# Nick-qsv/MLP-PPO-2PLY-P3

Hardware: AMD Instinct MI355X
Metric: self-play env steps/sec (whole node) + 2-ply evals/sec at batch=65536 (higher is better)
Workload: dtype int8 boards / fp32-equivalent policy MLP (split-f16 MFMA); 1 GPU; C3: B=65536 games/GPU PPO rollout step (policy 198->128->{500,1} + masked sample + env.step, rollout rows stored to an HBM ring); global_batch=65536, games_per_gpu=65536, max_legal_moves=500, parallelism=dp1 (independent game shards), streams_per_gpu=4, step_fork=False

## Files before the change

mlp-ppo-2ply-p3_amd/csrc/bg_engine.h:

```cpp
#pragma once
#include <hip/hip_runtime.h>
#include <stdint.h>
#include <stdlib.h>
#include <string>

#include "bg_core.h"
#include "../../include/bgx.h"

namespace bg {

template <int LOG> constexpr int cap_fast() { return (7 << LOG) / 8; }
constexpr int kLogSlotsSlow = 17;
constexpr int kCapSlow = (7 << kLogSlotsSlow) / 8;
constexpr int kSlowWaves = 32;
constexpr int kMtWords = 640;

constexpr int R_CUR = 52, R_ROLL0 = 53, R_ROLL1 = 54, R_OVER = 55, R_MATCH = 56, R_S0 = 57, R_S1 = 58,
              R_NEED = 59, R_NM0 = 60, R_NM1 = 61, R_FLAGS = 62;
constexpr int NEED_NONE = 0, NEED_ROLL = 1, NEED_RESET = 2;

__device__ __forceinline__ int lane_id() { return threadIdx.x & 63; }
__device__ __forceinline__ int rd(int bv, int i) { return __builtin_amdgcn_readlane(bv, i); }
__device__ __forceinline__ int wr(int bv, int i, int v) { return lane_id() == i ? v : bv; }
__device__ __forceinline__ uint32_t ufl(uint32_t v) { return __builtin_amdgcn_readfirstlane(v); }
// ... 78 lines not shown
            #pragma unroll
            for (int r = 0; r < 10; ++r) {
                const uint32_t h0 = __umulhi(0xD2511F53u, c0), l0 = 0xD2511F53u * c0;
                const uint32_t h1 = __umulhi(0xCD9E8D57u, c2), l1 = 0xCD9E8D57u * c2;
                c0 = h1 ^ c1 ^ a0; c1 = l1; c2 = h0 ^ c3 ^ a1; c3 = l0;
                a0 += 0x9E3779B9u; a1 += 0xBB67AE85u;
            }
            blk0 = c0; blk1 = c1; blk2 = c2; blk3 = c3; blkid = b;
        }
        const uint32_t w = (uint32_t)(ctr & 3u);
        ++ctr;
        return w == 0 ? blk0 : w == 1 ? blk1 : w == 2 ? blk2 : blk3;
    }

    template <bool PHILOX_ONLY = false>
    __device__ int die() {
        used = true;
        for (;;) {
            const uint32_t x = (PHILOX_ONLY || mode == BGX_DICE_PHILOX ? next_philox() : next_mt()) & 7u;
            if (x <= 5u) return (int)x + 1;
        }
    }

    template <bool PHILOX_ONLY = false>
    __device__ void finish(uint64_t* ctr_out) {
        if (!used) return;
        if (PHILOX_ONLY || mode == BGX_DICE_PHILOX) {
            if (lane_id() == 0) *ctr_out = ctr;
            return;
        }
        if (twisted) {
            for (int j = lane_id(); j < 624; j += 64) mt[j] = sh[j];
        }
        if (lane_id() == 0) mt[624] = (uint32_t)idx;
    }
};

struct Args {
    uint8_t* lanes;
    uint64_t* moves;
    int32_t* n_total;
    uint32_t* mt;
    uint64_t* ctr;
    uint8_t* shared_rolls;
    int32_t* ovf_count;
    int32_t* ovf_queue;
    int32_t* err;
    int B, max_moves, dice_mode, auto_reset, match_length;
    uint32_t key0, key1;
    uint64_t* stamps;
    int cap_mid;
    int cap_main;
    int32_t* perm;
    uint8_t* cls;
    uint8_t* pre;
    int xcd;
    const uint8_t* starts;
};
constexpr int kStartOk = 63;

__device__ __forceinline__ int lane_of_block(const Args& A, int bi) {
    if (!A.xcd) return bi;
    const int r = bi & 127;
    return (bi & ~127) | ((r & 7) << 4) | (r >> 3);
}

constexpr int kClasses = 5;

constexpr uint64_t kCtrMask = (1ull << 48) - 1ull;

constexpr int kPreOver = 0x80;
__device__ __forceinline__ int pre_class(int bv) {
    if (rd(bv, R_OVER)) return kPreOver;
    const int nxt = 1 - rd(bv, R_CUR);
    const int l = lane_id();
    const int off = nxt * 24;
    const bool mine = l >= off && l < off + 24 && bv > 0;
    return __popcll(__ballot(mine)) + (rd(bv, 48 + nxt) > 0 ? 2 : 0);
}

__device__ __forceinline__ int predict_class(int pre, uint64_t ctr, uint32_t key0, uint32_t key1, uint32_t lane_no,
                                             uint32_t& cache) {
    cache = 0u;
    if (pre & kPreOver) return kClasses - 1;
    Rng r;
    const uint64_t c0 = ctr & kCtrMask;
    r.init_philox(c0, key0, key1, lane_no);
    const int a = r.die(), b = r.die();
    const uint64_t draws = r.ctr - c0;
    if (draws < 32) cache = 0x8000u | (uint32_t)a | ((uint32_t)b << 3) | ((uint32_t)draws << 6);
    if (a != b) return kClasses - 1;
    const int pts = pre;
    if (pts >= 10 && a <= 4) return 0;
    if ((pts >= 8 && a <= 5) || pts >= 10) return 1;
    return pts >= 5 ? 2 : 3;
}

template <int LOG, typename SlotPtr, int MEMO_KIND = 0, bool NO_DOUBLES = false>
__device__ __forceinline__ int run_movegen(int bv, int pl, int r0, int r1, uint64_t* out, int cap, SlotPtr tab,
                                           int cap_unique, int* total, bool* ovf, uint4* memo) {
    const bool dbl = r0 == r1;
    Gen<LOG, SlotPtr, MoveSink, MEMO_KIND> g;
    g.tab = tab; g.sink.out = out; g.sink.cap = cap; g.pl = pl; g.cap_unique = cap_unique;
    g.memo2 = memo && dbl ? memo : nullptr;
    g.memo3 = memo && dbl ? (MEMO_KIND != 0 ? memo : memo + (1 << kLogMemo2)) : nullptr;
    uint32_t blocked;
    const Node s0 = node_from_bytes(bv, pl, blocked);
    g.blocked = blocked;
    if (NO_DOUBLES) g.run_nd(s0, r0, r1);
    else g.run(s0, r0, r1);
    *ovf = g.ovf;
    *total = g.count;
    return g.count < cap ? g.count : cap;
}

template <int DICE = -1>
__device__ __forceinline__ bool roll_lane(int& bv, int gi, const Args& A, uint32_t* mt_scratch, uint64_t* ctr_io,
                                          int& r0, int& r1) {
    const int need = rd(bv, R_NEED);
    if (need == NEED_NONE) return false;
// ... 75 lines not shown
}

__device__ __forceinline__ int defer_lane(int bv, int gi, const Args& A) {
    if (lane_id() == 0) { const int q = atomicAdd(A.ovf_count, 1); A.ovf_queue[q] = gi; A.n_total[gi] = 0; }
    bv = wr(bv, R_NM0, 0);
    bv = wr(bv, R_NM1, 0);
    bv = wr(bv, R_FLAGS, rd(bv, R_FLAGS) | 1);
    return wr(bv, R_NEED, NEED_NONE);
}

template <int LOG, int MEMO_KIND = 0, bool NO_DOUBLES = false, int DICE = -1>
__device__ __forceinline__ int advance_lane(int bv, int gi, const Args& A, uint4* lds_tab, uint4* lds_memo,
                                            uint64_t* ctr_io) {
    int r0, r1;
    if (!roll_lane<DICE>(bv, gi, A, (uint32_t*)lds_tab, ctr_io, r0, r1)) return bv;
    if (NO_DOUBLES && r0 == r1) return defer_lane(bv, gi, A);
    return movegen_lane<LOG, MEMO_KIND, NO_DOUBLES>(bv, gi, A, r0, r1, lds_tab, lds_memo);
}

__device__ __forceinline__ void write_obs(int bv, float* obs_row) {
    const int cur = rd(bv, R_CUR);
    #pragma unroll
    for (int t = 0; t < 4; ++t) {
        const int f = lane_id() + 64 * t;
        const float v = feature_at(bv, f < 198 ? f : 197, cur);
        if (f < 198) obs_row[f] = v;
    }
}

__device__ __forceinline__ int apply_move_bytes(int bv, uint32_t mlo, uint32_t mhi, int pl) {
    mlo = opaque(mlo); mhi = opaque(mhi);
    const int l = lane_id();
    const uint32_t q = (uint32_t)(l - pl * 24);
    const uint32_t o = (uint32_t)(l - (24 - pl * 24));
    constexpr uint32_t kNone = 32u;
    const uint32_t my_src = q < 24u ? q : (l == 48 + pl ? (uint32_t)kBar : kNone);
    const uint32_t my_dst = q < 24u ? q : (l == 50 + pl ? (uint32_t)kOff : kNone);
    uint32_t ok = 1u, hits = 0u;
    int delta = 0;
    #pragma unroll
    for (int i = 0; i < 4; ++i) {
        const uint32_t e = (i < 2 ? mlo : mhi) >> (16 * (i & 1));
        ok &= e >> 15;
        const uint32_t src = e & 31u, dst = (e >> 5) & 31u;
        const int d = (int)(dst == my_dst) - (int)(src == my_src);
        delta += ok ? d : 0;
        hits |= (ok & (e >> 10)) << dst;
    }
    if (o < 24u) delta -= (int)((hits >> o) & 1u);
    if (l == 49 - pl) delta += __popc(hits);
    return bv + delta;
}

__device__ __forceinline__ int apply_lane(int bv, int gi, int action, const Args& A, float* reward, uint8_t* done,
                                          int32_t* info) {
    const int mover = rd(bv, R_CUR);
    int winner = -1, score = 0, kind = 0, dn = 0;
    float rew = 0.0f;
    if (rd(bv, R_OVER)) {
        bv = wr(bv, R_NEED, NEED_RESET);
        dn = 1; kind = 3;
    } else {
        const int n = rd(bv, R_NM0) | (rd(bv, R_NM1) << 8);
        if (n == 0) {
            bv = wr(bv, R_CUR, 1 - mover);
            bv = wr(bv, R_NEED, NEED_ROLL);
            kind = 1;
        } else {
            const int a = action < 0 ? action + A.max_moves : action;
            if (a < 0 || a >= n) {
                rew = -1.0f; kind = 2;
            } else {
                const uint64_t mv = A.moves[(size_t)gi * A.max_moves + a];
                bv = apply_move_bytes(bv, (uint32_t)mv, (uint32_t)(mv >> 32), mover);
                if (rd(bv, 50 + mover) == 15) {
                    const int opp = 1 - mover;
                    const bool opp_off0 = rd(bv, 50 + opp) == 0;
                    const int l = lane_id();
                    const int hl = mover == 0 ? 18 : 0;
                    const bool in_home = l >= opp * 24 + hl && l < opp * 24 + hl + 6 && bv > 0;
                    const bool bg = opp_off0 && (__ballot(in_home) != 0ull || rd(bv, 48 + opp) > 0);
                    score = bg ? 3 : (opp_off0 ? 2 : 1);
                    rew = bg ? 2.0f : (opp_off0 ? 1.5f : 1.0f);
                    winner = mover; dn = 1;
                    const int ns = rd(bv, R_S0 + mover) + score;
                    bv = wr(bv, R_S0 + mover, ns > 255 ? 255 : ns);
                    bv = wr(bv, R_OVER, 1);
                    if (ns >= A.match_length) bv = wr(bv, R_MATCH, 1);
                    if (A.auto_reset) bv = wr(bv, R_NEED, NEED_RESET);
                } else {
                    bv = wr(bv, R_CUR, 1 - mover);
                    bv = wr(bv, R_NEED, NEED_ROLL);
                }
            }
        }
    }
    if (lane_id() == 0) {
        reward[gi] = rew;
        done[gi] = (uint8_t)dn;
        if (info) info[gi] = mover | ((winner + 1) << 8) | (score << 16) | (kind << 24);
    }
    return bv;
}

__device__ __forceinline__ int load_rec(const Args& A, int gi) { return (int)A.lanes[(size_t)gi * 64 + lane_id()]; }
__device__ __forceinline__ void store_rec(const Args& A, int gi, int bv) { A.lanes[(size_t)gi * 64 + lane_id()] = (uint8_t)bv; }


}

struct DeviceBuf {
    void* p = nullptr;
    size_t cap = 0;
    hipError_t reserve(size_t bytes, int slack_num, hipStream_t stream, size_t keep_bytes) {
        if (cap >= bytes) return hipSuccess;
        hipError_t err = hipStreamSynchronize(stream);
        if (err != hipSuccess) return err;
        const size_t ncap = bytes + bytes * (size_t)slack_num / 100;
        void* np = nullptr;
        if ((err = hipMalloc(&np, ncap)) != hipSuccess) return err;
        if (p && keep_bytes) {
            err = hipMemcpyAsync(np, p, keep_bytes, hipMemcpyDeviceToDevice, stream);
            if (err == hipSuccess) err = hipStreamSynchronize(stream);
            if (err != hipSuccess) { (void)hipFree(np); return err; }
        }
        void* old = p;
        p = np;
        cap = ncap;
        return old ? hipFree(old) : hipSuccess;
    }
};

struct bgx_engine {
    bool step_debug{false};
    int device{0};
    bg::Args a{};
    uint4* slow_tables{nullptr};
    int slow_waves{bg::kSlowWaves};
    int32_t* perm{nullptr};
    bool perm_valid{false};
    int32_t* order_cnt{nullptr};
    hipStream_t step_side{nullptr};
    hipEvent_t step_ev[4]{};
    bool order_pending{false};
    bool step_fork{true};
    int32_t* ovf_base{nullptr};
    int ovf_parity{0};
    bool ovf_next_zeroed{false};
    uint64_t seed{0};
    uint8_t* starts{nullptr};
    DeviceBuf search_ws;
    DeviceBuf search_pool;
    hipStream_t search_side{nullptr};
    hipEvent_t search_ev[5]{};
    float search_ms[2]{};
    DeviceBuf oneply_ws;
    hipEvent_t use_ev{nullptr};
    hipStream_t use_stream{nullptr};
    bool use_valid{false};
};

inline hipError_t join_order(bgx_engine* e, hipStream_t s) {
    if (!e->order_pending) return hipSuccess;
    const hipError_t err = hipStreamWaitEvent(s, e->step_ev[3], 0);
    if (err == hipSuccess) e->order_pending = false;
    return err;
}

struct EngineCall {
    bgx_engine* e;
    hipStream_t s;
    bool entered = false, captured = false;
    hipError_t err;
    EngineCall(bgx_engine* e_, hipStream_t s_, bool join = false) : e(e_), s(s_), err(hipSetDevice(e_->device)) {
        if (err != hipSuccess) return;
        entered = true;
        hipStreamCaptureStatus cs = hipStreamCaptureStatusNone;
        if (hipStreamIsCapturing(s, &cs) == hipSuccess && cs != hipStreamCaptureStatusNone) captured = true;
        if (!captured && e->use_valid && e->use_stream != s) err = hipStreamWaitEvent(s, e->use_ev, 0);
        if (err == hipSuccess && join) err = join_order(e, s);
    }
    ~EngineCall() {
        if (!entered) return;
        if (captured) { e->use_valid = false; return; }
        if (!e->use_ev && hipEventCreateWithFlags(&e->use_ev, hipEventDisableTiming) != hipSuccess) {
            e->use_ev = nullptr;
            e->use_valid = false;
            return;
        }
        e->use_valid = hipEventRecord(e->use_ev, s) == hipSuccess;
        e->use_stream = s;
    }
};
// ... 1 lines not shown
```

mlp-ppo-2ply-p3_amd/csrc/bg_engine.hip:

```cpp
#include <hip/hip_runtime.h>
#include <stdio.h>
#include <stdint.h>
#include <string.h>
#include <stdlib.h>
#include <algorithm>
#include <cmath>
#include <mutex>
#include <string>
#include <vector>

#include "bg_engine.h"
#include "bg_rollout.h"
#include "bg_debug.h"
#include "bg_host.h"
#include <map>

using namespace bg;

namespace {

constexpr int kMaxRegions = BGX_MAX_COPY_REGIONS;
using namespace bg;

template <int PHASE, int LOG, int MEMO, bool NO_DOUBLES = false, int DICE = -1>
__device__ __forceinline__ void step_lane(const Args& A, int gi, uint4* tab, uint4* memo, const int32_t* actions,
                                          float* obs, float* reward, uint8_t* done, int32_t* info) {
    const uint64_t t0 = A.stamps ? __builtin_amdgcn_s_memrealtime() : 0;
    int bv = load_rec(A, gi);
    const int act = PHASE != 2 ? (int)ufl((uint32_t)actions[gi]) : 0;
    uint64_t ctr = (DICE >= 0 ? DICE : A.dice_mode) == BGX_DICE_PHILOX ? A.ctr[gi] : 0;
    if (PHASE != 2) bv = apply_lane(bv, gi, act, A, reward, done, info);
    if (PHASE != 1) {
        bv = advance_lane<LOG, MEMO == 2 ? 2 : 0, NO_DOUBLES, DICE>(bv, gi, A, tab, memo, &ctr);
        if (obs) write_obs(bv, obs + (size_t)gi * 198);
    }
    store_rec(A, gi, bv);
    if (PHASE == 0 && A.pre) {
        const int p = pre_class(bv);
        if (lane_id() == 0) A.pre[gi] = (uint8_t)p;
    }
    if (A.stamps && lane_id() == 0) {
        A.stamps[2 * gi] = t0;
        A.stamps[2 * gi + 1] = __builtin_amdgcn_s_memrealtime();
    }
}

template <int PHASE, int LOG, int MEMO = 1, bool NO_DOUBLES = false, int WPE = 1, int DICE = -1>
__global__ __launch_bounds__(64) __attribute__((amdgpu_waves_per_eu(WPE))) void k_step(Args A, const int32_t* actions, float* obs, float* reward, uint8_t* done,
                                             int32_t* info, int base) {
    __shared__ uint4 tab[1 << LOG];
    __shared__ uint4 memo_[MEMO == 1 ? kMemoSlots : 1];
    uint4* memo = MEMO == 1 ? memo_ : MEMO == 2 ? tab : nullptr;
    const int bi = (int)blockIdx.x + base;
    const int gi = A.perm ? (int)ufl((uint32_t)A.perm[bi]) : lane_of_block(A, bi);
    step_lane<PHASE, LOG, MEMO, NO_DOUBLES, DICE>(A, gi, tab, memo, actions, obs, reward, done, info);
}

template <int LOG>
__global__ __launch_bounds__(64) void k_reset(Args A, const uint8_t* lane_mask, float* obs, int mark_only) {
    __shared__ uint4 tab[1 << LOG];
    __shared__ uint4 memo[kMemoSlots];
    const int gi = blockIdx.x;
    int bv = load_rec(A, gi);
    uint64_t ctr = A.dice_mode == BGX_DICE_PHILOX ? A.ctr[gi] : 0;
    const bool sel = lane_mask == nullptr || ufl(lane_mask[gi]) != 0u;
    if (sel) bv = wr(bv, R_NEED, NEED_RESET);
    if (!mark_only) {
        bv = advance_lane<LOG>(bv, gi, A, tab, memo, &ctr);
        if (obs) write_obs(bv, obs + (size_t)gi * 198);
        if (A.pre) {
            const int p = pre_class(bv);
            if (lane_id() == 0) A.pre[gi] = (uint8_t)p;
        }
    }
    store_rec(A, gi, bv);
}

constexpr int kXcd = 8, kRun = 16;
__device__ __forceinline__ int order_class(const uint8_t* cls, int i, int B) {
    return i < B ? min((int)cls[i], kClasses - 1) : kClasses;
}

constexpr int kCountThreads = 256;
__global__ __launch_bounds__(kCountThreads) void k_order_count(const uint8_t* pre, uint8_t* cls, uint64_t* ctr, uint32_t key0,
                                                      uint32_t key1, int32_t* cnt, int B, int32_t* zero_next,
                                                      int xcd) {
    __shared__ int sc[kXcd][kClasses];
    const int t = threadIdx.x, i = blockIdx.x * kCountThreads + t, w = t >> 6;
    if (blockIdx.x == 0 && t < 4) zero_next[t] = 0;
    if (t < kXcd * kClasses) sc[t / kClasses][t % kClasses] = 0;
    __syncthreads();
    int c = kClasses;
    if (i < B) {
        const int p = (int)pre[i];
        const uint64_t cv = (p & kPreOver) ? 0ull : ctr[i];
        uint32_t cache;
        c = predict_class(p, cv, key0, key1, (uint32_t)i, cache);
        if (cache) ctr[i] = (cv & kCtrMask) | ((uint64_t)cache << 48);
        cls[i] = (uint8_t)c;
    }
    #pragma unroll
    for (int k = 0; k < kClasses; ++k) {
        const uint64_t m = __ballot(c == k);
        if (xcd) {
            if ((t & 63) < 4) {
                const int s = t & 3;
                const int n = __popcll(m & (0xFFFFull << (16 * s)));
                if (n) atomicAdd(&sc[(4 * w + s) & 7][k], n);
            }
        } else if ((t & 63) == 0 && m) {
            atomicAdd(&sc[0][k], __popcll(m));
        }
    }
    __syncthreads();
    if (t < kXcd * kClasses) cnt[blockIdx.x * kXcd * kClasses + t] = sc[t / kClasses][t % kClasses];
}

__global__ __launch_bounds__(1024) void k_order_scatter(const uint8_t* cls, const int32_t* cnt, int32_t* perm, int B,
                                                        int ncnt, int xcd) {
    constexpr int NC = kXcd * kClasses, STRIPES = 1024 / NC, PER = 1024 / kCountThreads;
    __shared__ int tot[NC], pre[NC], wsum[16][4][kClasses];
    const int t = threadIdx.x, b = blockIdx.x, w = t >> 6, l = t & 63;
    if (t < NC) { tot[t] = 0; pre[t] = 0; }
    __syncthreads();
    if (t < NC * STRIPES) {
        const int k = t % NC;
        int a_tot = 0, a_pre = 0;
        for (int j = t / NC; j < ncnt; j += STRIPES) {
            const int v = cnt[j * NC + k];
            a_tot += v;
            a_pre += j < b * PER ? v : 0;
        }
        if (a_tot) atomicAdd(&tot[k], a_tot);
        if (a_pre) atomicAdd(&pre[k], a_pre);
    }
    const int i = b * 1024 + t;
    const int c = order_class(cls, i, B);
    const int s = xcd ? (l >> 4) : 0;
    const uint64_t seg = xcd ? (0xFFFFull << (16 * s)) : ~0ull;
    int rank = 0;
    #pragma unroll
    for (int k = 0; k < kClasses; ++k) {
        const uint64_t m = __ballot(c == k);
        if (c == k) rank = __popcll(m & seg & ((1ull << l) - 1ull));
        if (l < 4) wsum[w][l][k] = __popcll(m & (xcd ? (0xFFFFull << (16 * l)) : (l == 0 ? ~0ull : 0ull)));
    }
    __syncthreads();
    if (c < kClasses) {
        const int x = xcd ? ((4 * w + s) & 7) : 0;
        int pos = pre[x * kClasses + c] + rank;
        for (int k = 0; k < c; ++k) pos += tot[x * kClasses + k];
        for (int v = xcd ? (w & 1) : 0; v < w; v += xcd ? 2 : 1) pos += wsum[v][s][c];
        perm[xcd ? pos * kXcd + x : pos] = i;
    }
}

__global__ __launch_bounds__(64) void k_shared_dice(Args A) {
    __shared__ uint32_t sh[640];
    Rng rng;
    rng.init_mt(A.mt, sh);
    for (int base = 0; base < A.B; base += 64) {
        const int j = base + lane_id();
        const int needv = j < A.B ? (int)A.lanes[(size_t)j * 64 + R_NEED] : 0;
        const int cnt = A.B - base < 64 ? A.B - base : 64;
        for (int t = 0; t < cnt; ++t) {
            const int need = __builtin_amdgcn_readlane(needv, t);
            if (need == NEED_NONE) continue;
            int r0, r1, starter = 0;
            if (need == NEED_RESET) {
                int a, b;
                do { a = rng.die(); b = rng.die(); } while (a == b);
                starter = a < b ? 1 : 0;
                do { r0 = rng.die(); r1 = rng.die(); } while (r0 == r1);
            } else {
                r0 = rng.die(); r1 = rng.die();
            }
            if (lane_id() == 0) {
                uint8_t* sr = A.shared_rolls + (size_t)(base + t) * 4;
                sr[0] = (uint8_t)r0; sr[1] = (uint8_t)r1; sr[2] = (uint8_t)starter;
            }
        }
    }
    rng.finish(nullptr);
}

template <int LOG>
__global__ __launch_bounds__(64) void k_movegen(const int8_t* boards, const uint8_t* players, const uint8_t* dice,
                                                int n, int cap, int16_t* nmoves, int32_t* ntotal, uint64_t* moves,
                                                int32_t* ovf_count, int32_t* ovf_queue, int cap_unique) {
    __shared__ uint4 tab[1 << LOG];
    __shared__ uint4 memo[kMemoSlots];
    const int gi = blockIdx.x;
    const int l = lane_id();
    const int bv = l < 52 ? (int)boards[(size_t)gi * 52 + l] : 0;
    const int pl = (int)ufl(players[gi]);
    const int r0 = (int)ufl(dice[2 * gi]), r1 = (int)ufl(dice[2 * gi + 1]);
    int total;
    bool ovf;
    int nm = run_movegen<LOG>(bv, pl, r0, r1, moves + (size_t)gi * cap, cap, tab, cap_unique, &total, &ovf, memo);
    if (ovf) {
        if (l == 0) { const int q = atomicAdd(ovf_count, 1); ovf_queue[q] = gi; }
        nm = 0; total = 0;
    }
    if (l == 0) { nmoves[gi] = (int16_t)nm; if (ntotal) ntotal[gi] = total; }
}

// ... 376 lines not shown
        lq = luck_q(lane_luck[i]);
        res = winner == (int)(starts[(size_t)i * 64 + R_CUR] & 1) ? score : -score;
    }
    if (dn) lane_luck[i] = 0.0f;
    for_each_group(fin, g, [&](int gl, bool mine, uint64_t m) {
        const long long v = mine ? lq : 0;
        int64_t* row = luck_tally + (size_t)gl * 4;
        tally_add(row, BGX_ROLLOUT_LUCK, wave_sum(v));
        tally_add(row, BGX_ROLLOUT_LUCK2, wave_sum(v * v));
        tally_add(row, BGX_ROLLOUT_RESLUCK, wave_sum(mine ? res * lq : 0));
        tally_add(row, BGX_ROLLOUT_LUCK_GAMES, (long long)__popcll(m));
    });
}

__device__ __forceinline__ uint64_t mix64(uint64_t x) {
    x ^= x >> 33; x *= 0xFF51AFD7ED558CCDull;
    x ^= x >> 33; x *= 0xC4CEB9FE1A85EC53ull;
    x ^= x >> 33;
    return x;
}

__global__ __launch_bounds__(256) void k_random_act(const uint8_t* recs, int n, uint64_t seed, uint32_t step,
                                                    int32_t* act) {
    const int i = blockIdx.x * 256 + threadIdx.x;
    if (i >= n) return;
    const uint32_t cnt = (uint32_t)recs[(size_t)i * 64 + R_NM0] | ((uint32_t)recs[(size_t)i * 64 + R_NM1] << 8);
    const uint64_t h = mix64(mix64(seed ^ 0x9E3779B97F4A7C15ull) + (((uint64_t)step << 32) | (uint32_t)i));
    act[i] = (int32_t)(((h >> 32) * (uint64_t)cnt) >> 32);
}

thread_local std::string g_err;

}

int bgx_internal_fail(hipError_t e, int code) {
    g_err = hipGetErrorString(e);
    return code;
}
void bgx_set_error(const char* msg) { g_err = msg; }
static std::mutex g_dbg_mu;
static std::map<std::string, std::string> g_dbg;
std::string bgx_dbg(const char* name) {
    std::lock_guard<std::mutex> g(g_dbg_mu);
    const auto it = g_dbg.find(name);
    return it == g_dbg.end() ? std::string() : it->second;
}
long long bgx_dbg_int(const char* name, long long dflt) {
    const std::string v = bgx_dbg(name);
    return v.empty() ? dflt : strtoll(v.c_str(), nullptr, 10);
}

#define LAUNCH_LOG(K, grid, s, ...) hipLaunchKernelGGL(K<9>, grid, dim3(64), 0, s, __VA_ARGS__)

static void launch_order(bgx_engine* e, hipStream_t s) {
    const int nblk = (e->a.B + 1023) / 1024, ncnt = (e->a.B + kCountThreads - 1) / kCountThreads;
    hipLaunchKernelGGL(k_order_count, dim3(ncnt), dim3(kCountThreads), 0, s, e->a.pre, e->a.cls, e->a.ctr, e->a.key0, e->a.key1,
                       e->order_cnt, e->a.B, e->ovf_base + 4 * (e->ovf_parity ^ 1), e->a.xcd);
    e->ovf_next_zeroed = true;
    hipLaunchKernelGGL(k_order_scatter, dim3(nblk), dim3(1024), 0, s, e->a.cls, e->order_cnt, e->perm, e->a.B, ncnt,
                       e->a.xcd);
    e->perm_valid = true;
}

struct StepIo {
    const int32_t* actions;
    float *obs, *reward;
    uint8_t* done;
    int32_t* info;
};

static void launch_heavy(hipStream_t s, const Args& a, int grid, const StepIo& io) {
    if (grid <= 0) return;
    if (a.dice_mode == BGX_DICE_PHILOX)
        hipLaunchKernelGGL((k_step<0, 9, 0, false, 1, BGX_DICE_PHILOX>), dim3(grid), dim3(64), 0, s, a, io.actions,
                           io.obs, io.reward, io.done, io.info, 0);
    else
        hipLaunchKernelGGL((k_step<0, 9, 0>), dim3(grid), dim3(64), 0, s, a, io.actions, io.obs, io.reward, io.done,
                           io.info, 0);
}

static void launch_light(hipStream_t s, const Args& a, int heavy, const StepIo& io) {
    hipLaunchKernelGGL((k_step<0, 8, 0, true, 1, BGX_DICE_PHILOX>), dim3(a.B - heavy), dim3(64), 0, s, a, io.actions,
                       io.obs, io.reward, io.done, io.info, heavy);
}

static int heavy_grid(int B, bool xcd) {
    const double g = B / 6.0 + 4.0 * std::sqrt(B * 5.0 / 36.0) + 32.0;
    int h = g >= B ? B : (int)g;
    if (xcd) h = (h + 7) & ~7;
    return h > B ? B : h;
}

static int slow_path(bgx_engine* e, hipStream_t s, int src, const int8_t* boards, const uint8_t* players,
                     const uint8_t* dice, int cap, int16_t* nm, int32_t* nt, uint64_t* moves) {
    if (src == 0)
        hipLaunchKernelGGL(k_movegen_over<0>, dim3(e->slow_waves), dim3(64), 0, s, e->a, boards, players, dice, cap,
                           nm, nt, moves, e->slow_tables);
    else
        hipLaunchKernelGGL(k_movegen_over<1>, dim3(e->slow_waves), dim3(64), 0, s, e->a, boards, players, dice, cap,
                           nm, nt, moves, e->slow_tables);
    return bgx_launch_status();
}

struct EngineBuf {
    void** p;
    size_t bytes;
    bool zero;
};
static std::vector<EngineBuf> engine_bufs(bgx_engine* e, bool stamps, bool order) {
    Args& A = e->a;
    const size_t B = (size_t)A.B;
    const bool shared = A.dice_mode == BGX_DICE_MT_SHARED;
    return {
        {(void**)&A.lanes, B * 64, true},
        {(void**)&A.moves, B * (size_t)A.max_moves * 8, false},
        {(void**)&A.n_total, B * 4, true},
        {(void**)&A.mt, (A.dice_mode == BGX_DICE_MT_LANE ? B : 1) * kMtWords * 4, false},
        {(void**)&A.ctr, B * 8, true},
        {(void**)&A.shared_rolls, B * 4, false},
        {(void**)&e->ovf_base, 32, true},
        {(void**)&A.ovf_queue, B * 4, false},
        {(void**)&A.err, 16, true},
        {(void**)&e->starts, shared ? 0 : B * 64, false},
        {(void**)&e->slow_tables, (size_t)kSlowWaves * ((size_t)16 << kLogSlotsSlow), false},
        {(void**)&A.stamps, stamps ? B * 16 : 0, false},
        {(void**)&e->perm, order ? B * 4 : 0, false},
        {(void**)&A.cls, order ? B : 0, true},
        {(void**)&A.pre, order ? B : 0, true},
        {(void**)&e->order_cnt, order ? (B / kCountThreads + 1) * kXcd * kClasses * 4 : 0, false},
    };
}

static hipError_t fresh_ovf_counters(bgx_engine* e, hipStream_t s, bool rotate) {
    if (rotate && e->ovf_next_zeroed) {
        e->ovf_parity ^= 1;
        e->a.ovf_count = e->ovf_base + 4 * e->ovf_parity;
        e->ovf_next_zeroed = false;
        return hipSuccess;
    }
    return hipMemsetAsync(e->a.ovf_count, 0, 16, s);
}

static void step_shared_dice(const Args& A, const StepIo& io, hipStream_t s) {
    hipLaunchKernelGGL((k_step<1, 9>), dim3(A.B), dim3(64), 0, s, A, io.actions, io.obs, io.reward, io.done, io.info, 0);
    hipLaunchKernelGGL(k_shared_dice, dim3(1), dim3(64), 0, s, A);
    hipLaunchKernelGGL((k_step<2, 9>), dim3(A.B), dim3(64), 0, s, A, io.actions, io.obs, io.reward, io.done, io.info, 0);
}

static int order_on_side(bgx_engine* e, hipStream_t s) {
    BGX_CK(hipEventRecord(e->step_ev[2], s));
    BGX_CK(hipStreamWaitEvent(e->step_side, e->step_ev[2], 0));
    launch_order(e, e->step_side);
    BGX_CK(hipEventRecord(e->step_ev[3], e->step_side));
    e->order_pending = true;
    return BGX_OK;
}

static int step_lane_dice(bgx_engine* e, const StepIo& io, hipStream_t s) {
    Args a = e->a;
    a.perm = e->perm_valid ? e->perm : nullptr;
    const int heavy = a.perm ? heavy_grid(a.B, a.xcd != 0) : a.B;
    if (heavy < a.B && e->step_fork) {
        if (!e->step_side) {
            BGX_CK(hipStreamCreateWithFlags(&e->step_side, hipStreamNonBlocking));
            for (hipEvent_t& ev : e->step_ev) BGX_CK(hipEventCreateWithFlags(&ev, hipEventDisableTiming));
        }
        BGX_CK(hipEventRecord(e->step_ev[0], s));
        BGX_CK(hipStreamWaitEvent(e->step_side, e->step_ev[0], 0));
        launch_heavy(s, a, heavy, io);
        launch_light(e->step_side, a, heavy, io);
        BGX_CK(hipEventRecord(e->step_ev[1], e->step_side));
        if (a.cls) {
            const int rc = order_on_side(e, s);
            if (rc != BGX_OK) return rc;
        }
        BGX_CK(hipStreamWaitEvent(s, e->step_ev[1], 0));
    } else {
        launch_heavy(s, a, heavy, io);
        if (heavy < a.B) launch_light(s, a, heavy, io);
        if (a.cls) launch_order(e, s);
    }
    return BGX_OK;
}

static int step_debug_dump(bgx_engine* e, hipStream_t s) {
    const Args& A = e->a;
    int32_t q[2] = {0, 0};
    BGX_CK(hipMemcpyAsync(q, A.ovf_count, 8, hipMemcpyDeviceToHost, s));
    BGX_CK(hipStreamSynchronize(s));
    fprintf(stderr, "[bgx step] overflow queue %d of %d lanes\n", q[0], A.B);
    for (int i = 0; i < q[0] && i < 4; ++i) {
        int32_t gi = 0;
        uint8_t rec[64];
        BGX_CK(hipMemcpy(&gi, A.ovf_queue + i, 4, hipMemcpyDeviceToHost));
        BGX_CK(hipMemcpy(rec, A.lanes + (size_t)gi * 64, 64, hipMemcpyDeviceToHost));
        int own = 0, outside = 0;
        const int pl = rec[52];
        for (int p = 0; p < 24; ++p) {
            own += rec[pl * 24 + p] > 0;
            if (!(pl == 0 ? p >= 18 : p < 6)) outside += rec[pl * 24 + p];
        }
        fprintf(stderr, "   lane %d pl %d roll %d-%d points %d outside %d bar %d off %d n %d\n", gi, pl, rec[53],
                rec[54], own, outside, rec[48 + pl], rec[50 + pl], rec[60] | (rec[61] << 8));
    }
    return BGX_OK;
}

#include "bg_bearoff.h"

extern "C" {

int bgx_engine_create(int device, int32_t batch, int32_t max_moves, uint64_t seed, int32_t dice_mode,
                      int32_t auto_reset, int32_t match_length, bgx_engine** out) {
    if (!out || batch <= 0 || max_moves <= 0 || max_moves > 32767 || dice_mode < 0 || dice_mode > 2)
        return BGX_EINVAL;
    BGX_CK(hipSetDevice(device));
    bgx_engine* e = new bgx_engine();
    e->device = device;
    e->seed = seed;
    Args& A = e->a;
    A.B = batch; A.max_moves = max_moves; A.dice_mode = dice_mode; A.auto_reset = auto_reset ? 1 : 0;
    A.match_length = match_length;
    A.key0 = (uint32_t)seed; A.key1 = (uint32_t)(seed >> 32);
    A.xcd = batch % 128 == 0 && bgx_dbg_int("BGX_XCD", 1) != 0 ? 1 : 0;
    e->step_debug = !bgx_dbg("BGX_STEP_DEBUG").empty();
    A.cap_mid = (int)std::min<long long>(std::max<long long>(bgx_dbg_int("BGX_TIER1_CAP", cap_fast<kLogMid>()), 1),
                                         cap_fast<kLogMid>());
    A.cap_main = (int)std::min<long long>(std::max<long long>(bgx_dbg_int("BGX_MOVEGEN_CAP", cap_fast<9>()), 1),
                                          cap_fast<9>());
    const bool stamps = !bgx_dbg("BGX_STAMPS").empty();
    const bool order = dice_mode == BGX_DICE_PHILOX && bgx_dbg_int("BGX_ORDER", 1) != 0;
    hipError_t err = hipSuccess;
    for (const EngineBuf& b : engine_bufs(e, stamps, order))
        if (err == hipSuccess && b.bytes) err = hipMalloc(b.p, b.bytes);
    A.ovf_count = e->ovf_base;
    if (err != hipSuccess) { bgx_engine_destroy(e); return bgx_internal_fail(err, BGX_ENOMEM); }
    for (const EngineBuf& b : engine_bufs(e, stamps, order)) {
        if (b.zero && b.bytes && hipMemset(*b.p, 0, b.bytes) != hipSuccess) {
            bgx_engine_destroy(e);
            return bgx_internal_fail(hipGetLastError());
        }
    }
    std::vector<uint32_t> seeds((size_t)batch);
    for (size_t i = 0; i < seeds.size(); ++i) seeds[i] = (uint32_t)(seed + i);
    int rc = bgx_engine_seed(e, seeds.data(), seed);
    if (rc != BGX_OK) { bgx_engine_destroy(e); return rc; }
    *out = e;
    return BGX_OK;
}

int bgx_engine_join(bgx_engine* e, void* stream) {
    if (!e) return BGX_EINVAL;
    EngineCall call(e, (hipStream_t)stream, true);
    BGX_CK(call.err);
    return BGX_OK;
}

int bgx_engine_order(bgx_engine* e, int32_t* perm_host, uint8_t* cls_host, uint64_t* ctr_host, void* stream) {
    if (!e) return BGX_EINVAL;
    if ((perm_host || cls_host) && (!e->a.cls || !e->perm_valid)) return BGX_EINVAL;
    hipStream_t s = (hipStream_t)stream;
    const size_t B = (size_t)e->a.B;
    {
        EngineCall call(e, s, true);
        BGX_CK(call.err);
        if (perm_host) BGX_CK(hipMemcpyAsync(perm_host, e->perm, B * 4, hipMemcpyDeviceToHost, s));
        if (cls_host) BGX_CK(hipMemcpyAsync(cls_host, e->a.cls, B, hipMemcpyDeviceToHost, s));
        if (ctr_host) BGX_CK(hipMemcpyAsync(ctr_host, e->a.ctr, B * 8, hipMemcpyDeviceToHost, s));
    }
    BGX_CK(hipStreamSynchronize(s));
    return BGX_OK;
}

int bgx_engine_set_fork(bgx_engine* e, int32_t fork, void* stream) {
    if (!e) return BGX_EINVAL;
    EngineCall call(e, (hipStream_t)stream, !fork);
    BGX_CK(call.err);
    e->step_fork = fork != 0;
    return BGX_OK;
}

int bgx_engine_destroy(bgx_engine* e) {
    if (!e) return BGX_EINVAL;
    (void)hipSetDevice(e->device);
    if (e->use_valid) (void)hipEventSynchronize(e->use_ev);
    if (e->use_ev) (void)hipEventDestroy(e->use_ev);
    for (const EngineBuf& b : engine_bufs(e, true, true)) if (*b.p) (void)hipFree(*b.p);
    for (const DeviceBuf* b : {&e->search_ws, &e->search_pool, &e->oneply_ws}) if (b->p) (void)hipFree(b->p);
    for (hipEvent_t ev : e->search_ev) if (ev) (void)hipEventDestroy(ev);
    for (hipEvent_t ev : e->step_ev) if (ev) (void)hipEventDestroy(ev);
    if (e->step_side) (void)hipStreamDestroy(e->step_side);
    if (e->search_side) (void)hipStreamDestroy(e->search_side);
    delete e;
    return BGX_OK;
}

int bgx_engine_seed(bgx_engine* e, const uint32_t* seeds_host, uint64_t philox_seed) {
    if (!e || !seeds_host) return BGX_EINVAL;
    BGX_CK(hipSetDevice(e->device));
    Args& A = e->a;
    BGX_CK(hipDeviceSynchronize());
    A.key0 = (uint32_t)philox_seed; A.key1 = (uint32_t)(philox_seed >> 32);
    BGX_CK(hipMemset(A.ctr, 0, (size_t)A.B * 8));
    if (A.dice_mode == BGX_DICE_PHILOX) {
        BGX_CK(hipDeviceSynchronize());
        return BGX_OK;
    }
    const int n = A.dice_mode == BGX_DICE_MT_LANE ? A.B : 1;
    uint32_t* dseeds = nullptr;
    BGX_CK(hipMalloc(&dseeds, (size_t)n * 4));
    hipError_t err = hipMemcpy(dseeds, seeds_host, (size_t)n * 4, hipMemcpyHostToDevice);
    if (err == hipSuccess) {
        hipLaunchKernelGGL(k_mt_seed, dim3((n + 255) / 256), dim3(256), 0, 0, A.mt, dseeds, n);
        err = hipGetLastError();
    }
    if (err == hipSuccess) err = hipDeviceSynchronize();
    (void)hipFree(dseeds);
    BGX_CK(err);
// ... 8 lines not shown
    if (lane < 0 || lane >= A.B) return BGX_EINVAL;
    BGX_CK(hipSetDevice(e->device));
    BGX_CK(hipDeviceSynchronize());
    uint32_t* dev = A.mt + (size_t)lane * kMtWords;
    if (set) BGX_CK(hipMemcpy(dev, state_host, 625 * 4, hipMemcpyHostToDevice));
    else BGX_CK(hipMemcpy(state_host, dev, 625 * 4, hipMemcpyDeviceToHost));
    return BGX_OK;
}

#ifdef BGX_COUNTERS
extern "C" int bgx_debug_counters(unsigned long long* out16) {
    BGX_CK(hipDeviceSynchronize());
    constexpr size_t n = 16 * (size_t)bg::kCntSlots;
    std::vector<unsigned long long> h(n), z(n, 0ull);
    BGX_CK(hipMemcpyFromSymbol(h.data(), HIP_SYMBOL(bg::g_cnt), n * 8));
    for (int i = 0; i < 16; ++i) {
        out16[i] = 0;
        for (int k = 0; k < bg::kCntSlots; ++k) out16[i] += h[(size_t)i * bg::kCntSlots + k];
    }
    BGX_CK(hipMemcpyToSymbol(HIP_SYMBOL(bg::g_cnt), z.data(), n * 8));
    return BGX_OK;
}
#endif

extern "C" int bgx_debug_stamps(bgx_engine* e, uint64_t* host_out) {
    if (!e || !host_out || !e->a.stamps) return BGX_EINVAL;
    BGX_CK(hipDeviceSynchronize());
    BGX_CK(hipMemcpy(host_out, e->a.stamps, (size_t)e->a.B * 16, hipMemcpyDeviceToHost));
    return BGX_OK;
}

int bgx_engine_buffers(bgx_engine* e, bgx_buffers* out) {
    if (!e || !out) return BGX_EINVAL;
    out->lanes = e->a.lanes; out->moves = e->a.moves; out->n_total = e->a.n_total;
    out->batch = e->a.B; out->max_moves = e->a.max_moves;
    return BGX_OK;
}

int bgx_reset(bgx_engine* e, const uint8_t* lane_mask_dev, float* obs_dev, void* stream) {
    if (!e) return BGX_EINVAL;
    hipStream_t s = (hipStream_t)stream;
    Args& A = e->a;
    EngineCall call(e, s, true);
    BGX_CK(call.err);
    BGX_CK(fresh_ovf_counters(e, s, true));
    if (A.dice_mode == BGX_DICE_MT_SHARED) {
        LAUNCH_LOG(k_reset, dim3(A.B), s, A, lane_mask_dev, obs_dev, 1);
        hipLaunchKernelGGL(k_shared_dice, dim3(1), dim3(64), 0, s, A);
        LAUNCH_LOG(k_reset, dim3(A.B), s, A, nullptr, obs_dev, 0);
    } else {
        LAUNCH_LOG(k_reset, dim3(A.B), s, A, lane_mask_dev, obs_dev, 0);
    }
    BGX_CK_LAUNCH();
    if (A.cls) {
        launch_order(e, s);
    }
    return slow_path(e, s, 0, nullptr, nullptr, nullptr, 0, nullptr, nullptr, nullptr);
}

int bgx_step(bgx_engine* e, const int32_t* actions_dev, float* obs_dev, float* reward_dev, uint8_t* done_dev,
             int32_t* info_dev, void* stream) {
    if (!e || !actions_dev || !reward_dev || !done_dev) return BGX_EINVAL;
    hipStream_t s = (hipStream_t)stream;
    const StepIo io{actions_dev, obs_dev, reward_dev, done_dev, info_dev};
    EngineCall call(e, s, true);
    BGX_CK(call.err);
    BGX_CK(fresh_ovf_counters(e, s, true));
    if (e->a.dice_mode == BGX_DICE_MT_SHARED) {
        step_shared_dice(e->a, io, s);
    } else {
        const int rc = step_lane_dice(e, io, s);
        if (rc != BGX_OK) return rc;
    }
    BGX_CK_LAUNCH();
    const int rc = slow_path(e, s, 0, nullptr, nullptr, nullptr, 0, nullptr, nullptr, nullptr);
    if (e->step_debug) {
        const int drc = step_debug_dump(e, s);
        if (drc != BGX_OK) return drc;
    }
    return rc;
}

int bgx_movegen(bgx_engine* e, const int8_t* boards52_dev, const uint8_t* players_dev, const uint8_t* dice_dev,
                int32_t n, int32_t max_moves, int16_t* n_moves_dev, int32_t* n_total_dev, uint64_t* moves_dev,
                void* stream) {
    if (!e || n < 0 || max_moves <= 0 || !boards52_dev || !players_dev || !dice_dev || !n_moves_dev || !moves_dev)
        return BGX_EINVAL;
    if (n > e->a.B) return BGX_EINVAL;
    if (n == 0) return BGX_OK;
    hipStream_t s = (hipStream_t)stream;
    EngineCall call(e, s);
    BGX_CK(call.err);
    BGX_CK(fresh_ovf_counters(e, s, false));
    LAUNCH_LOG(k_movegen, dim3(n), s, boards52_dev, players_dev, dice_dev, n, max_moves, n_moves_dev, n_total_dev,
               moves_dev, e->a.ovf_count, e->a.ovf_queue, e->a.cap_main);
    BGX_CK_LAUNCH();
    return slow_path(e, s, 1, boards52_dev, players_dev, dice_dev, max_moves, n_moves_dev, n_total_dev, moves_dev);
}

int bgx_encode(const int8_t* boards52_dev, const uint8_t* players_dev, int32_t n, float* out_dev, void* stream) {
    if (n < 0 || (n > 0 && (!boards52_dev || !players_dev || !out_dev))) return BGX_EINVAL;
    if (n == 0) return BGX_OK;
    hipLaunchKernelGGL(k_encode, dim3(n), dim3(64), 0, (hipStream_t)stream, boards52_dev, players_dev, n, out_dev);
    BGX_CK_LAUNCH();
    return BGX_OK;
}

int bgx_encode_records_ex(const uint8_t* records_dev, int32_t n, int32_t dtype, int32_t width, void* out_dev,
                          void* stream) {
// ... 255 lines not shown
```

Measured before the change: 517.7 million env steps/s.

## Defer order scatter into a step-time gather that packs per-lane step inputs

The order scatter kernel is replaced by a gather kernel that runs at the start of the next step, once actions are known. Besides writing the permutation, it writes a 32-byte per-slot record holding the lane index, action, the chosen move and the dice counter. The step kernels then load that record with scalar loads instead of doing separate dependent reads of perm, actions, ctr and the large moves array. This removes scattered global loads from the step's critical path, at the cost of an extra buffer write per lane and moving the ordering work onto the step stream.

```diff
diff --git a/mlp-ppo-2ply-p3_amd/csrc/bg_engine.h b/mlp-ppo-2ply-p3_amd/csrc/bg_engine.h
--- a/mlp-ppo-2ply-p3_amd/csrc/bg_engine.h
+++ b/mlp-ppo-2ply-p3_amd/csrc/bg_engine.h
@@ -154,6 +154,7 @@
     int cap_mid;
     int cap_main;
     int32_t* perm;
+    const uint8_t* blk;
     uint8_t* cls;
     uint8_t* pre;
     int xcd;
@@ -168,6 +169,8 @@
 }
 
 constexpr int kClasses = 5;
+
+constexpr int kBlkBytes = 32;
 
 constexpr uint64_t kCtrMask = (1ull << 48) - 1ull;
 
@@ -349,8 +352,9 @@
     return bv + delta;
 }
 
+template <bool HAVE_MV = false>
 __device__ __forceinline__ int apply_lane(int bv, int gi, int action, const Args& A, float* reward, uint8_t* done,
-                                          int32_t* info) {
+                                          int32_t* info, uint64_t chosen = 0) {
     const int mover = rd(bv, R_CUR);
     int winner = -1, score = 0, kind = 0, dn = 0;
     float rew = 0.0f;
@@ -368,7 +372,7 @@
             if (a < 0 || a >= n) {
                 rew = -1.0f; kind = 2;
             } else {
-                const uint64_t mv = A.moves[(size_t)gi * A.max_moves + a];
+                const uint64_t mv = HAVE_MV ? chosen : A.moves[(size_t)gi * A.max_moves + a];
                 bv = apply_move_bytes(bv, (uint32_t)mv, (uint32_t)(mv >> 32), mover);
                 if (rd(bv, 50 + mover) == 15) {
                     const int opp = 1 - mover;
@@ -435,7 +439,8 @@
     uint4* slow_tables{nullptr};
     int slow_waves{bg::kSlowWaves};
     int32_t* perm{nullptr};
-    bool perm_valid{false};
+    uint8_t* blk{nullptr};
+    bool gather_due{false};
     int32_t* order_cnt{nullptr};
     hipStream_t step_side{nullptr};
     hipEvent_t step_ev[4]{};
diff --git a/mlp-ppo-2ply-p3_amd/csrc/bg_engine.hip b/mlp-ppo-2ply-p3_amd/csrc/bg_engine.hip
--- a/mlp-ppo-2ply-p3_amd/csrc/bg_engine.hip
+++ b/mlp-ppo-2ply-p3_amd/csrc/bg_engine.hip
@@ -22,14 +22,30 @@
 constexpr int kMaxRegions = BGX_MAX_COPY_REGIONS;
 using namespace bg;
 
-template <int PHASE, int LOG, int MEMO, bool NO_DOUBLES = false, int DICE = -1>
-__device__ __forceinline__ void step_lane(const Args& A, int gi, uint4* tab, uint4* memo, const int32_t* actions,
+template <int PHASE, int LOG, int MEMO, bool NO_DOUBLES = false, int DICE = -1, bool BLK = false>
+__device__ __forceinline__ void step_lane(const Args& A, int at, uint4* tab, uint4* memo, const int32_t* actions,
                                           float* obs, float* reward, uint8_t* done, int32_t* info) {
     const uint64_t t0 = A.stamps ? __builtin_amdgcn_s_memrealtime() : 0;
-    int bv = load_rec(A, gi);
-    const int act = PHASE != 2 ? (int)ufl((uint32_t)actions[gi]) : 0;
-    uint64_t ctr = (DICE >= 0 ? DICE : A.dice_mode) == BGX_DICE_PHILOX ? A.ctr[gi] : 0;
-    if (PHASE != 2) bv = apply_lane(bv, gi, act, A, reward, done, info);
+    int gi = at, bv, act;
+    uint64_t ctr, chosen = 0;
+    if (BLK) {
+        const uint8_t* b = A.blk + (size_t)at * kBlkBytes;
+        typedef uint32_t u32x4 __attribute__((ext_vector_type(4)));
+        typedef uint32_t u32x2 __attribute__((ext_vector_type(2)));
+        const uintptr_t hp = (uintptr_t)b;
+        const u32x4 h = *(const __attribute__((address_space(4))) u32x4*)hp;
+        const u32x2 c = *(const __attribute__((address_space(4))) u32x2*)(hp + 16);
+        asm volatile("s_mov_b32 %0, %1" : "=s"(gi) : "s"(h.x));
+        bv = load_rec(A, gi);
+        act = (int)h.y;
+        chosen = (uint64_t)h.z | ((uint64_t)h.w << 32);
+        ctr = (uint64_t)c.x | ((uint64_t)c.y << 32);
+    } else {
+        bv = load_rec(A, gi);
+        act = PHASE != 2 ? (int)ufl((uint32_t)actions[gi]) : 0;
+        ctr = (DICE >= 0 ? DICE : A.dice_mode) == BGX_DICE_PHILOX ? A.ctr[gi] : 0;
+    }
+    if (PHASE != 2) bv = apply_lane<BLK>(bv, gi, act, A, reward, done, info, chosen);
     if (PHASE != 1) {
         bv = advance_lane<LOG, MEMO == 2 ? 2 : 0, NO_DOUBLES, DICE>(bv, gi, A, tab, memo, &ctr);
         if (obs) write_obs(bv, obs + (size_t)gi * 198);
@@ -45,15 +61,15 @@
     }
 }
 
-template <int PHASE, int LOG, int MEMO = 1, bool NO_DOUBLES = false, int WPE = 1, int DICE = -1>
+template <int PHASE, int LOG, int MEMO = 1, bool NO_DOUBLES = false, int WPE = 1, int DICE = -1, bool BLK = false>
 __global__ __launch_bounds__(64) __attribute__((amdgpu_waves_per_eu(WPE))) void k_step(Args A, const int32_t* actions, float* obs, float* reward, uint8_t* done,
                                              int32_t* info, int base) {
     __shared__ uint4 tab[1 << LOG];
     __shared__ uint4 memo_[MEMO == 1 ? kMemoSlots : 1];
     uint4* memo = MEMO == 1 ? memo_ : MEMO == 2 ? tab : nullptr;
     const int bi = (int)blockIdx.x + base;
-    const int gi = A.perm ? (int)ufl((uint32_t)A.perm[bi]) : lane_of_block(A, bi);
-    step_lane<PHASE, LOG, MEMO, NO_DOUBLES, DICE>(A, gi, tab, memo, actions, obs, reward, done, info);
+    const int at = BLK ? bi : A.perm ? (int)ufl((uint32_t)A.perm[bi]) : lane_of_block(A, bi);
+    step_lane<PHASE, LOG, MEMO, NO_DOUBLES, DICE, BLK>(A, at, tab, memo, actions, obs, reward, done, info);
 }
 
 template <int LOG>
@@ -116,11 +132,24 @@
     if (t < kXcd * kClasses) cnt[blockIdx.x * kXcd * kClasses + t] = sc[t / kClasses][t % kClasses];
 }
 
-__global__ __launch_bounds__(1024) void k_order_scatter(const uint8_t* cls, const int32_t* cnt, int32_t* perm, int B,
-                                                        int ncnt, int xcd) {
-    constexpr int NC = kXcd * kClasses, STRIPES = 1024 / NC, PER = 1024 / kCountThreads;
-    __shared__ int tot[NC], pre[NC], wsum[16][4][kClasses];
+constexpr int kGatherThreads = kCountThreads;
+template <bool BLOCKS>
+__global__ __launch_bounds__(kGatherThreads) void k_step_gather(const uint8_t* cls, const int32_t* cnt, int32_t* perm,
+                                                                int B, int ncnt, int xcd, const uint64_t* moves,
+                                                                const uint64_t* ctr, const int32_t* actions,
+                                                                int max_moves, uint8_t* blk) {
+    constexpr int T = kGatherThreads, NC = kXcd * kClasses, STRIPES = T / NC, PER = T / kCountThreads;
+    __shared__ int tot[NC], pre[NC], wsum[T / 64][4][kClasses];
     const int t = threadIdx.x, b = blockIdx.x, w = t >> 6, l = t & 63;
+    const int i = b * T + t;
+    int act = 0;
+    uint64_t cv = 0, mv = 0;
+    if (BLOCKS && i < B) {
+        act = actions[i];
+        cv = ctr[i];
+        const int a = act < 0 ? act + max_moves : act;
+        if (a >= 0 && a < max_moves) mv = moves[(size_t)i * max_moves + a];
+    }
     if (t < NC) { tot[t] = 0; pre[t] = 0; }
     __syncthreads();
     if (t < NC * STRIPES) {
@@ -134,7 +163,6 @@
         if (a_tot) atomicAdd(&tot[k], a_tot);
         if (a_pre) atomicAdd(&pre[k], a_pre);
     }
-    const int i = b * 1024 + t;
     const int c = order_class(cls, i, B);
     const int s = xcd ? (l >> 4) : 0;
     const uint64_t seg = xcd ? (0xFFFFull << (16 * s)) : ~0ull;
@@ -151,7 +179,13 @@
         int pos = pre[x * kClasses + c] + rank;
         for (int k = 0; k < c; ++k) pos += tot[x * kClasses + k];
         for (int v = xcd ? (w & 1) : 0; v < w; v += xcd ? 2 : 1) pos += wsum[v][s][c];
-        perm[xcd ? pos * kXcd + x : pos] = i;
+        const int p = xcd ? pos * kXcd + x : pos;
+        perm[p] = i;
+        if (BLOCKS) {
+            uint4* o = (uint4*)(blk + (size_t)p * kBlkBytes);
+            o[0] = make_uint4((uint32_t)i, (uint32_t)act, (uint32_t)mv, (uint32_t)(mv >> 32));
+            o[1] = make_uint4((uint32_t)cv, (uint32_t)(cv >> 32), 0u, 0u);
+        }
     }
 }
 
@@ -634,14 +668,23 @@
 
 #define LAUNCH_LOG(K, grid, s, ...) hipLaunchKernelGGL(K<9>, grid, dim3(64), 0, s, __VA_ARGS__)
 
-static void launch_order(bgx_engine* e, hipStream_t s) {
-    const int nblk = (e->a.B + 1023) / 1024, ncnt = (e->a.B + kCountThreads - 1) / kCountThreads;
+static void launch_count(bgx_engine* e, hipStream_t s) {
+    const int ncnt = (e->a.B + kCountThreads - 1) / kCountThreads;
     hipLaunchKernelGGL(k_order_count, dim3(ncnt), dim3(kCountThreads), 0, s, e->a.pre, e->a.cls, e->a.ctr, e->a.key0, e->a.key1,
                        e->order_cnt, e->a.B, e->ovf_base + 4 * (e->ovf_parity ^ 1), e->a.xcd);
     e->ovf_next_zeroed = true;
-    hipLaunchKernelGGL(k_order_scatter, dim3(nblk), dim3(1024), 0, s, e->a.cls, e->order_cnt, e->perm, e->a.B, ncnt,
-                       e->a.xcd);
-    e->perm_valid = true;
+    e->gather_due = true;
+}
+
+static void launch_gather(bgx_engine* e, hipStream_t s, const int32_t* actions) {
+    const Args& A = e->a;
+    const int nblk = (A.B + kGatherThreads - 1) / kGatherThreads, ncnt = (A.B + kCountThreads - 1) / kCountThreads;
+    if (actions)
+        hipLaunchKernelGGL(k_step_gather<true>, dim3(nblk), dim3(kGatherThreads), 0, s, A.cls, e->order_cnt, e->perm, A.B,
+                           ncnt, A.xcd, A.moves, A.ctr, actions, A.max_moves, e->blk);
+    else
+        hipLaunchKernelGGL(k_step_gather<false>, dim3(nblk), dim3(kGatherThreads), 0, s, A.cls, e->order_cnt, e->perm, A.B,
+                           ncnt, A.xcd, nullptr, nullptr, nullptr, 0, nullptr);
 }
 
 struct StepIo {
@@ -653,7 +696,10 @@
 
 static void launch_heavy(hipStream_t s, const Args& a, int grid, const StepIo& io) {
     if (grid <= 0) return;
-    if (a.dice_mode == BGX_DICE_PHILOX)
+    if (a.blk)
+        hipLaunchKernelGGL((k_step<0, 9, 0, false, 1, BGX_DICE_PHILOX, true>), dim3(grid), dim3(64), 0, s, a, io.actions,
+                           io.obs, io.reward, io.done, io.info, 0);
+    else if (a.dice_mode == BGX_DICE_PHILOX)
         hipLaunchKernelGGL((k_step<0, 9, 0, false, 1, BGX_DICE_PHILOX>), dim3(grid), dim3(64), 0, s, a, io.actions,
                            io.obs, io.reward, io.done, io.info, 0);
     else
@@ -662,7 +708,7 @@
 }
 
 static void launch_light(hipStream_t s, const Args& a, int heavy, const StepIo& io) {
-    hipLaunchKernelGGL((k_step<0, 8, 0, true, 1, BGX_DICE_PHILOX>), dim3(a.B - heavy), dim3(64), 0, s, a, io.actions,
+    hipLaunchKernelGGL((k_step<0, 8, 0, true, 1, BGX_DICE_PHILOX, true>), dim3(a.B - heavy), dim3(64), 0, s, a, io.actions,
                        io.obs, io.reward, io.done, io.info, heavy);
 }
 
@@ -707,6 +753,7 @@
         {(void**)&e->slow_tables, (size_t)kSlowWaves * ((size_t)16 << kLogSlotsSlow), false},
         {(void**)&A.stamps, stamps ? B * 16 : 0, false},
         {(void**)&e->perm, order ? B * 4 : 0, false},
+        {(void**)&e->blk, order ? B * kBlkBytes : 0, false},
         {(void**)&A.cls, order ? B : 0, true},
         {(void**)&A.pre, order ? B : 0, true},
         {(void**)&e->order_cnt, order ? (B / kCountThreads + 1) * kXcd * kClasses * 4 : 0, false},
@@ -732,7 +779,7 @@
 static int order_on_side(bgx_engine* e, hipStream_t s) {
     BGX_CK(hipEventRecord(e->step_ev[2], s));
     BGX_CK(hipStreamWaitEvent(e->step_side, e->step_ev[2], 0));
-    launch_order(e, e->step_side);
+    launch_count(e, e->step_side);
     BGX_CK(hipEventRecord(e->step_ev[3], e->step_side));
     e->order_pending = true;
     return BGX_OK;
@@ -740,7 +787,12 @@
 
 static int step_lane_dice(bgx_engine* e, const StepIo& io, hipStream_t s) {
     Args a = e->a;
-    a.perm = e->perm_valid ? e->perm : nullptr;
+    if (a.cls && e->gather_due) {
+        launch_gather(e, s, io.actions);
+        e->gather_due = false;
+        a.perm = e->perm;
+        a.blk = e->blk;
+    }
     const int heavy = a.perm ? heavy_grid(a.B, a.xcd != 0) : a.B;
     if (heavy < a.B && e->step_fork) {
         if (!e->step_side) {
@@ -760,7 +812,7 @@
     } else {
         launch_heavy(s, a, heavy, io);
         if (heavy < a.B) launch_light(s, a, heavy, io);
-        if (a.cls) launch_order(e, s);
+        if (a.cls) launch_count(e, s);
     }
     return BGX_OK;
 }
@@ -840,12 +892,16 @@
 
 int bgx_engine_order(bgx_engine* e, int32_t* perm_host, uint8_t* cls_host, uint64_t* ctr_host, void* stream) {
     if (!e) return BGX_EINVAL;
-    if ((perm_host || cls_host) && (!e->a.cls || !e->perm_valid)) return BGX_EINVAL;
+    if ((perm_host || cls_host) && (!e->a.cls || !e->gather_due)) return BGX_EINVAL;
     hipStream_t s = (hipStream_t)stream;
     const size_t B = (size_t)e->a.B;
     {
         EngineCall call(e, s, true);
         BGX_CK(call.err);
+        if (perm_host) {
+            launch_gather(e, s, nullptr);
+            BGX_CK_LAUNCH();
+        }
         if (perm_host) BGX_CK(hipMemcpyAsync(perm_host, e->perm, B * 4, hipMemcpyDeviceToHost, s));
         if (cls_host) BGX_CK(hipMemcpyAsync(cls_host, e->a.cls, B, hipMemcpyDeviceToHost, s));
         if (ctr_host) BGX_CK(hipMemcpyAsync(ctr_host, e->a.ctr, B * 8, hipMemcpyDeviceToHost, s));
@@ -960,9 +1016,7 @@
         LAUNCH_LOG(k_reset, dim3(A.B), s, A, lane_mask_dev, obs_dev, 0);
     }
     BGX_CK_LAUNCH();
-    if (A.cls) {
-        launch_order(e, s);
-    }
+    if (A.cls) launch_count(e, s);
     return slow_path(e, s, 0, nullptr, nullptr, nullptr, 0, nullptr, nullptr, nullptr);
 }
 
```

Measured after the change: 541.6 million env steps/s, median of 6. 1.05x the previous value.
